# NivekNey/polars-matmul

Hardware: AMD Instinct MI355X
Metric: cosine top-k queries/sec (higher is better)
Workload: dtype f32

## Files before the change

polars-matmul_amd/csrc/pmm_kernels.hip:

```cpp
#include "pmm_device.h"

#include <algorithm>

#include <hip/hip_runtime.h>
#include <math.h>
#include <stdint.h>

#include <type_traits>

namespace pmm {

hipError_t launch_norms_f32(const float *a, int64_t rows, int64_t d, int64_t ld, int squared,
                            float *out, float *inv, hipStream_t s) {
  if (rows <= 0) return hipSuccess;
  const int64_t threads = rows * 8;
  const unsigned grid = (unsigned)((threads + 255) / 256);
  norms_kernel<float><<<grid, 256, 0, s>>>(a, rows, d, ld, squared, out, inv);
  return hipGetLastError();
}
hipError_t launch_norms_pair_f32(const float *q, int64_t m, int64_t ldq, float *qout, const float *c,
                                 int64_t n, int64_t ldc, float *cout, float *cinv, int64_t d, int squared,
                                 hipStream_t s, void *zero, size_t zero_bytes) {
  const unsigned gq = (unsigned)((m * 8 + 255) / 256), gc = (unsigned)((n * 8 + 255) / 256);
  if (zero_bytes % 16 != 0 || ((uintptr_t)zero & 15)) return hipErrorInvalidValue;
// ... 1701 lines not shown
      z1_bytes % 16)
    return hipErrorInvalidValue;
  PrologueArgs a{};
  a.q = q;
  a.ldq = ldq;
  a.m = m;
  a.c = c;
  a.ldc = ldc;
  a.n = n;
  a.d = d;
  a.dp = dp;
  a.ns = ns;
  a.k = k;
  a.squared = metric == kMetricEuclidean;
  a.qn = qn;
  a.cn = cn;
  a.cinv = cn + n;
  a.gthr = gthr;
  a.z0 = (uint4 *)z0;
  a.z1 = (uint4 *)z1;
  a.z0n = (int64_t)(z0_bytes / 16);
  a.z1n = (int64_t)(z1_bytes / 16);
#ifdef PMM_LAB
  a.ablate = getenv("PMM_PROLOGUE_ABLATE") ? atoi(getenv("PMM_PROLOGUE_ABLATE")) : 0;
#endif
  const char *le = getenv("PMM_SEED_LDS");
  a.lds_seed = (ns <= 256 && dp <= seedk::kLdsMaxDp && le && atoi(le) == 1) ? 1 : 0;
  const bool xf = metric != kMetricDot;
  const char *me = getenv("PMM_SEED_MFMA");
  const bool mfma_ok = ns == seedm::NSM && dp <= seedm::kMaxDp && !a.lds_seed && n >= seedm::NSM;
  a.mfma_seed = (mfma_ok && (me ? atoi(me) != 0 : PMM_SEED_MFMA_DEFAULT != 0)) ? 1 : 0;
  if (a.mfma_seed) {
    a.sblocks = (unsigned)((m + seedm::RM - 1) / seedm::RM);
    constexpr int T = seedm::NT;
    a.qblocks = xf ? (unsigned)((m * 8 + T - 1) / T) : 0u;
    a.cblocks = (xf && corpus_norms) ? (unsigned)((n * 8 + T - 1) / T) : 0u;
    a.zblocks = (unsigned)std::max<int64_t>(1, std::min<int64_t>((a.z0n + a.z1n + T - 1) / T, 16));
    const unsigned grid = a.sblocks + a.qblocks + a.cblocks + a.zblocks;
    if (metric == kMetricCosine) return launch_prologue_mfma_t<kMetricCosine>(a, grid, s);
    if (metric == kMetricDot) return launch_prologue_mfma_t<kMetricDot>(a, grid, s);
    return launch_prologue_mfma_t<kMetricEuclidean>(a, grid, s);
  }
  a.sblocks = (unsigned)((m + seedk::RQ - 1) / seedk::RQ);
  unsigned grid;
  if (a.lds_seed) {
    a.qblocks = 0u;
    grid = std::max<unsigned>(a.sblocks, (xf && corpus_norms) ? (unsigned)((n + 63) / 64) : 1u);
    a.cper = (n + grid - 1) / grid;
    a.cblocks = (xf && corpus_norms) ? 1u : 0u;
    a.zblocks = 0u;
  } else {
    a.qblocks = xf ? (unsigned)((m * 8 + 255) / 256) : 0u;
    a.cblocks = (xf && corpus_norms) ? (unsigned)((n * 8 + 255) / 256) : 0u;
    a.zblocks = (unsigned)std::max<int64_t>(1, std::min<int64_t>((a.z0n + a.z1n + 255) / 256, 64));
    grid = a.sblocks + a.qblocks + a.cblocks + a.zblocks;
  }
  if (metric == kMetricCosine) return launch_prologue_t<kMetricCosine>(a, grid, s);
  if (metric == kMetricDot) return launch_prologue_t<kMetricDot>(a, grid, s);
  return launch_prologue_t<kMetricEuclidean>(a, grid, s);
}

constexpr int kMergeRankMaxRows = 16384;
hipError_t launch_merge(const MergeArgs &a0, int loader, hipStream_t s) {
  if (a0.M <= 0) return hipSuccess;
  MergeArgs a = a0;
  static const int rank_env = getenv("PMM_MERGE_RANK") ? atoi(getenv("PMM_MERGE_RANK")) : -1;
  a.no_rank = rank_env == 0 || (rank_env < 0 && a.M > kMergeRankMaxRows);
  a.flags = getenv("PMM_MERGE_FLAGS") ? atoi(getenv("PMM_MERGE_FLAGS"))
                                     : (kMergeReverse | kMergePipelined | kMergeSplitRow);
  const bool sorted = loader == 1 && a.sorted && a.S <= 64 && a.k_out <= 256 && a.P <= 512 &&
                      !(getenv("PMM_MERGE_SORTED") && atoi(getenv("PMM_MERGE_SORTED")) == 0);
  static const int kp = getenv("PMM_KWAY_P") ? atoi(getenv("PMM_KWAY_P")) : 24;
  if (sorted && a.S >= 5 && a.S <= 8 && a.k_out <= 8 * (kp == 32 ? 32 : 24) &&
      !(getenv("PMM_MERGE_KWAY") && atoi(getenv("PMM_MERGE_KWAY")) == 0) &&
      (size_t)MPN(a.P) * 8 <= (size_t)64 * (kp == 32 ? 32 : 24) * 8) {
    static const int wpb = getenv("PMM_KWAY_WPB") ? atoi(getenv("PMM_KWAY_WPB")) : 4;
    const int rows_per_block = 8 * wpb;
    const unsigned grid = (unsigned)((a.M + rows_per_block - 1) / rows_per_block);
    if (kp != 32) {
      if (wpb == 4) (void)hipFuncSetAttribute((const void *)kway_merge_kernel<24>, hipFuncAttributeMaxDynamicSharedMemorySize, 160 * 1024);
      kway_merge_kernel<24><<<grid, 64 * wpb, (size_t)wpb * 64 * 24 * 8, s>>>(a);
    } else {
      if (wpb == 4) (void)hipFuncSetAttribute((const void *)kway_merge_kernel<32>, hipFuncAttributeMaxDynamicSharedMemorySize, 160 * 1024);
      kway_merge_kernel<32><<<grid, 64 * wpb, (size_t)wpb * 64 * 32 * 8, s>>>(a);
    }
    return hipGetLastError();
  }
  if (!(a.S >= 8 && a.k_out <= 64 && a.P <= 512 && !a.no_rank && a.ablate == 0) || sorted) a.flags &= ~kMergeSplitRow;
  const bool split = (a.flags & kMergeSplitRow) != 0;
  int wpb = (int)(65536 / merge_lds_bytes_per_wave(a.P));
  wpb = split ? 4 : (wpb < 1 ? 1 : (wpb > 4 ? 4 : wpb));
  const size_t lds = (size_t)wpb * merge_lds_bytes_per_wave(a.P) + (split ? 16 : 0);
  const unsigned grid = split ? (unsigned)a.M : (unsigned)((a.M + wpb - 1) / wpb);
  if (lds > 65536) {
    static bool attr_set[2] = {false, false};
    if (!attr_set[loader]) {
      const void *fn = loader == 0 ? (const void *)merge_kernel<0, false> : (const void *)merge_kernel<1, false>;
      hipError_t e = hipFuncSetAttribute(fn, hipFuncAttributeMaxDynamicSharedMemorySize, 160 * 1024);
      if (e != hipSuccess) return e;
      attr_set[loader] = true;
    }
  }
  if (sorted) {
    merge_kernel<1, false, true><<<grid, wpb * 64, lds, s>>>(a);
  } else if (split) {
    if (loader == 0) merge_kernel<0, true><<<grid, wpb * 64, lds, s>>>(a);
    else merge_kernel<1, true><<<grid, wpb * 64, lds, s>>>(a);
  } else {
    if (loader == 0) merge_kernel<0, false><<<grid, wpb * 64, lds, s>>>(a);
    else merge_kernel<1, false><<<grid, wpb * 64, lds, s>>>(a);
  }
  return hipGetLastError();
}


template <typename T>
__device__ __forceinline__ u64 score_key(T v, int metric);
template <>
__device__ __forceinline__ u64 score_key<float>(float v, int metric) {
  return (u64)okey32(metric == kMetricEuclidean ? -v : v);
}
template <>
__device__ __forceinline__ u64 score_key<double>(double v, int metric) {
  return okey64(metric == kMetricEuclidean ? -v : v);
}
template <typename T>
__device__ __forceinline__ T key_score(u64 k, int metric);
template <>
__device__ __forceinline__ float key_score<float>(u64 k, int metric) {
  const float v = dekey32((uint32_t)k);
  return metric == kMetricEuclidean ? 0.0f - v : v;
}
template <>
__device__ __forceinline__ double key_score<double>(u64 k, int metric) {
  const double v = dekey64(k);
  return metric == kMetricEuclidean ? 0.0 - v : v;
}

__device__ int ent_compact(Ent *scr, int cnt, int k, int P, Ent *Tv, bool *tfull, int lane) {
  for (int i = cnt + lane; i < P; i += 64) scr[i] = Ent{0ull, 0xFFFFFFFFu, 0u};
  wave_sync();
  wave_sort_desc_ent(scr, P, lane);
  if (cnt >= k) {
    *Tv = scr[k - 1];
    *tfull = true;
    cnt = k;
  }
  wave_sync();
  return cnt;
}

template <typename T>
__global__ __launch_bounds__(256) void rowselect_kernel(RowSelArgs a) {
  extern __shared__ __attribute__((aligned(16))) char smem[];
  const int lane = threadIdx.x & 63, wid = threadIdx.x >> 6;
  const int wpb = blockDim.x >> 6;
  const int row = blockIdx.x * wpb + wid;
  if (row >= a.rows) return;
  Ent *scr = (Ent *)smem + (size_t)wid * a.P;
  const T *src = (const T *)a.scores + (int64_t)row * a.lds;
  Ent Tv{0ull, 0xFFFFFFFFu, 0u};
  bool tfull = false;
  int cnt = 0;
  for (int i0 = 0; i0 < a.N; i0 += 64) {
    const int j = i0 + lane;
    Ent x{0ull, 0xFFFFFFFFu, 0u};
    bool keep = false;
    if (j < a.N) {
      x.key = score_key<T>(src[j], a.metric);
      x.idx = (uint32_t)j;
      keep = !tfull || ent_better(x, Tv);
    }
    const u64 m = __ballot(keep);
    const int pos = cnt + lanes_below(m);
    if (keep) scr[pos] = x;
    cnt += __popcll(m);
    if (cnt > a.P - 64) {
      wave_sync();
      cnt = ent_compact(scr, cnt, a.k, a.P, &Tv, &tfull, lane);
    }
  }
  wave_sync();
  const int P2 = min(a.P, next_pow2_dev(cnt));
  for (int i = cnt + lane; i < P2; i += 64) scr[i] = Ent{0ull, 0xFFFFFFFFu, 0u};
  wave_sync();
  wave_sort_desc_ent(scr, P2, lane);
  T *os = (T *)a.out_score;
  for (int j = lane; j < a.k; j += 64) {
    const Ent x = scr[j];
    a.out_idx[(int64_t)row * a.k + j] = x.idx + a.index_base;
    os[(int64_t)row * a.k + j] = key_score<T>(x.key, a.metric);
  }
}

hipError_t launch_rowselect(const RowSelArgs &a, hipStream_t s) {
  if (a.rows <= 0) return hipSuccess;
  const size_t per_wave = (size_t)a.P * sizeof(Ent);
  int wpb = (int)(65536 / per_wave);
  wpb = wpb < 1 ? 1 : (wpb > 4 ? 4 : wpb);
  const size_t lds = (size_t)wpb * per_wave;
  const unsigned grid = (unsigned)((a.rows + wpb - 1) / wpb);
  if (a.is_f64) rowselect_kernel<double><<<grid, wpb * 64, lds, s>>>(a);
  else rowselect_kernel<float><<<grid, wpb * 64, lds, s>>>(a);
  return hipGetLastError();
}

template <typename T>
__global__ void rowsort_build(const T *__restrict__ scores, int64_t lds, int rows, int N, int P2,
                              int metric, Ent *__restrict__ keys) {
  const int64_t t = (int64_t)blockIdx.x * blockDim.x + threadIdx.x;
  if (t >= (int64_t)rows * P2) return;
  const int r = (int)(t / P2), j = (int)(t % P2);
  Ent e{0ull, 0xFFFFFFFFu, 0u};
  if (j < N) {
    e.key = score_key<T>(scores[(int64_t)r * lds + j], metric);
    e.idx = (uint32_t)j;
  }
  keys[t] = e;
}
__global__ void rowsort_step(Ent *keys, int rows, int P2, int size, int stride) {
  const int64_t t = (int64_t)blockIdx.x * blockDim.x + threadIdx.x;
  const int64_t half = (int64_t)P2 >> 1;
  if (t >= (int64_t)rows * half) return;
  const int r = (int)(t / half), i = (int)(t % half);
  const int x0 = ((i & ~(stride - 1)) << 1) | (i & (stride - 1));
  const int x1 = x0 + stride;
  Ent *base = keys + (int64_t)r * P2;
  const Ent a = base[x0], b = base[x1];
  const bool desc = (x0 & size) == 0;
  if (desc ? ent_better(b, a) : ent_better(a, b)) {
    base[x0] = b;
    base[x1] = a;
  }
}
template <typename T>
__global__ void rowsort_extract(const Ent *__restrict__ keys, int rows, int P2, int k, int metric,
                                uint32_t index_base, uint32_t *__restrict__ out_idx,
                                T *__restrict__ out_score) {
  const int64_t t = (int64_t)blockIdx.x * blockDim.x + threadIdx.x;
  if (t >= (int64_t)rows * k) return;
  const int r = (int)(t / k), j = (int)(t % k);
  const Ent e = keys[(int64_t)r * P2 + j];
  out_idx[t] = e.idx + index_base;
  out_score[t] = key_score<T>(e.key, metric);
}

hipError_t launch_rowsort_global(const void *scores, int64_t lds, int rows, int N, int is_f64,
                                 int metric, void *keys_ws, int P2, int k, uint32_t index_base,
                                 uint32_t *out_idx, void *out_score, hipStream_t s) {
  if (rows <= 0) return hipSuccess;
  Ent *keys = (Ent *)keys_ws;
  const int64_t tot = (int64_t)rows * P2;
  const unsigned gb = (unsigned)((tot + 255) / 256);
  if (is_f64) rowsort_build<double><<<gb, 256, 0, s>>>((const double *)scores, lds, rows, N, P2, metric, keys);
  else rowsort_build<float><<<gb, 256, 0, s>>>((const float *)scores, lds, rows, N, P2, metric, keys);
  const unsigned gs = (unsigned)((tot / 2 + 255) / 256);
  for (int size = 2; size <= P2; size <<= 1)
    for (int stride = size >> 1; stride > 0; stride >>= 1)
      rowsort_step<<<gs, 256, 0, s>>>(keys, rows, P2, size, stride);
  const int64_t tk = (int64_t)rows * k;
  const unsigned ge = (unsigned)((tk + 255) / 256);
  if (is_f64) rowsort_extract<double><<<ge, 256, 0, s>>>(keys, rows, P2, k, metric, index_base, out_idx, (double *)out_score);
  else rowsort_extract<float><<<ge, 256, 0, s>>>(keys, rows, P2, k, metric, index_base, out_idx, (float *)out_score);
  return hipGetLastError();
}

__global__ __launch_bounds__(256) void screen_prep_kernel(const float *__restrict__ rel,
                                                          const unsigned *__restrict__ scal, int m, int dp,
                                                          float *__restrict__ eps, u64 *gthr, int seeded) {
  const int row = (int)(blockIdx.x * blockDim.x + threadIdx.x);
  if (row >= m) return;
  const float e = screen_eps(rel[row], __uint_as_float(scal[0]), dp);
  eps[row] = e;
  if (seeded) gthr[row] = screen_lower(gthr[row], e);
}
hipError_t launch_screen_prep(const float *rel, const unsigned *scal, int m, int dp, float *eps,
                              unsigned long long *gthr, int seeded, hipStream_t s) {
  if (m <= 0) return hipSuccess;
  screen_prep_kernel<<<(unsigned)((m + 255) / 256), 256, 0, s>>>(rel, scal, m, dp, eps, gthr, seeded);
  return hipGetLastError();
}

constexpr int kRescoreList = 512;

template <typename F>
__device__ __forceinline__ void rescore_each_entry(const ScreenFinishArgs &a, u64 *base, const unsigned *segs,
                                                   int nseg, F &&f) {
  const int tid = threadIdx.x, nt = blockDim.x;
  for (int t = 0; t < nseg; t++) {
    const unsigned e = segs[t];
    const int n = (int)(e & 1023u);
    u64 *seg = base + (int64_t)(e >> 10) * a.capg;
    for (int i0 = tid; i0 < n; i0 += 4 * nt) {
      u64 x[4];
#pragma unroll
      for (int j = 0; j < 4; j++) x[j] = i0 + j * nt < n ? seg[i0 + j * nt] : 0ull;
#pragma unroll
      for (int j = 0; j < 4; j++)
        if (i0 + j * nt < n) f(seg + i0 + j * nt, x[j]);
    }
  }
}

__global__ __launch_bounds__(256, 8) void screen_rescore_kernel(ScreenFinishArgs a) {
  extern __shared__ __attribute__((aligned(16))) char smem[];
  __shared__ __attribute__((aligned(16))) unsigned hist[256];
  __shared__ unsigned list[kRescoreList];
  __shared__ unsigned res[4], ln, emin;
  float *qs = (float *)smem;
  unsigned *segs = (unsigned *)(qs + a.dp);
  const int tid = threadIdx.x, nt = blockDim.x;
  const int row = (int)blockIdx.x;
  const float *qr = a.q + (int64_t)row * a.ldq;
  for (int i = 4 * tid; i < a.dp; i += 4 * nt) *(f32x4 *)(qs + i) = *(const f32x4 *)(qr + i);
  for (int i = tid; i < 256; i += nt) hist[i] = 0u;
  if (tid == 0) emin = ~0u, ln = 0u;
  __syncthreads();
  for (int s = tid; s < a.S; s += nt) {
    const unsigned n = min(a.cnt[(int64_t)row * a.S + s], (unsigned)a.capg);
    if (n) segs[atomicAdd(&ln, 1u)] = ((unsigned)s << 10) | n;
  }
  __syncthreads();
  const int nseg = (int)ln;
  const float qv = a.qn[row];
  const float eps = a.eps[row];
  const u64 T = screen_lower(a.gthr[row], eps);
  const u64 T1 = T ? T : 1ull;
  u64 *base = a.cand + (int64_t)row * a.S * a.capg;

  auto live = [&](u64 x) __attribute__((always_inline)) -> bool {
    return x >= T1 && ~(uint32_t)x < (uint32_t)a.N;
  };
  u64 P = 0ull;
  unsigned n_r = 0u, need = (unsigned)a.k;
  for (int shift = 56; shift >= 0; shift -= 8) {
    rescore_each_entry(a, base, segs, nseg, [&](u64 *, u64 x) __attribute__((always_inline)) {
      if (live(x) && (shift == 56 || ((x ^ P) >> (shift + 8)) == 0ull))
        atomicAdd(&hist[(unsigned)(x >> shift) & 255u], 1u);
    });
    __syncthreads();
    if (tid < 64) {
      const uint4 h = ((const uint4 *)hist)[tid];
      ((uint4 *)hist)[tid] = make_uint4(0u, 0u, 0u, 0u);
      const unsigned own = h.x + h.y + h.z + h.w;
      unsigned suf = own;
#pragma unroll
      for (int o = 1; o < 64; o <<= 1) {
        const unsigned t = __shfl_down(suf, o);
        if (tid + o < 64) suf += t;
      }
      if (tid == 0) {
        res[0] = res[1] = res[2] = 0u;
        if (shift == 56) res[3] = suf;
      }
      unsigned above = suf - own;
      if (above < need && suf >= need) {
        unsigned b = 3u, in_bin = h.w;
        if (above + in_bin < need) above += in_bin, in_bin = h.z, b = 2u;
        if (above + in_bin < need) above += in_bin, in_bin = h.y, b = 1u;
        if (above + in_bin < need) above += in_bin, in_bin = h.x, b = 0u;
        res[0] = 4u * (unsigned)tid + b;
        res[1] = need - above;
        res[2] = in_bin;
      }
    }
    __syncthreads();
    P |= (u64)res[0] << shift;
    need = res[1];
    if (shift == 56) n_r = res[3];
    if (res[2] == need) break;
  }
  const int max_rounds = (int)(((int64_t)a.S * a.capg + kRescoreList - 1) / kRescoreList) + 1;
  unsigned done = 0u;
  for (int ph = n_r > (unsigned)a.k ? 1 : 2; ph <= 2; ph++) {
    const bool last = ph == 2;
    u64 thr = P;
    if (last) {
      __syncthreads();
      const u64 E = screen_lower((u64)emin << 32, eps);
      thr = E > T1 ? E : T1;
    }
    for (int r = 0; r < max_rounds; r++) {
      __syncthreads();
      if (tid == 0) ln = 0u;
      __syncthreads();
      rescore_each_entry(a, base, segs, nseg, [&](u64 *p, u64 x) __attribute__((always_inline)) {
        if (x == 0ull) return;
        const uint32_t lw = (uint32_t)x;
        if (!(lw & 0x80000000u)) return;
        if (x < thr || !live(x)) {
          if (last) *p = 0ull;
          return;
        }
        const unsigned pos = atomicAdd(&ln, 1u);
        if (pos < (unsigned)kRescoreList) list[pos] = (unsigned)(p - base);
      });
      __syncthreads();
      const unsigned n = ln;
      const bool more = n > (unsigned)kRescoreList;
      const int cnt = more ? kRescoreList : (int)n;
      for (int t = tid; t < cnt; t += nt) {
        u64 *p = base + list[t];
        const uint32_t col = ~(uint32_t)*p;
        const float *cr = a.c + (int64_t)col * a.ldc;
        float acc = 0.0f;
        for (int k0 = 0; k0 < a.dp; k0 += 32) {
          f32x4 v[8];
#pragma unroll
          for (int j = 0; j < 8; j++) v[j] = *(const f32x4 *)(cr + k0 + 4 * j);
#pragma unroll
          for (int j = 0; j < 8; j++) {
            const f32x4 q4 = *(const f32x4 *)(qs + k0 + 4 * j);
            acc = fmaf(q4[0], v[j][0], acc);
            acc = fmaf(q4[1], v[j][1], acc);
            acc = fmaf(q4[2], v[j][2], acc);
            acc = fmaf(q4[3], v[j][3], acc);
          }
        }
        const uint32_t key = okey32(exact_score<kMetricCosine>(acc, qv, a.cn[col]));
        if (!last) atomicMin(&emin, key);
        *p = ((u64)key << 32) | (u64)col;
        done++;
      }
      if (!more) break;
    }
  }
  __syncthreads();
  rescore_each_entry(a, base, segs, nseg, [&](u64 *p, u64 x) __attribute__((always_inline)) {
    if (x != 0ull && !((uint32_t)x & 0x80000000u)) *p = (x & 0xFFFFFFFF00000000ull) | (u64)(~(uint32_t)x);
  });
  if (a.stat) {
    __syncthreads();
    if (tid == 0) ln = 0u;
    __syncthreads();
    atomicAdd(&ln, done);
    __syncthreads();
    if (tid == 0) {
      atomicAdd(a.stat, ln);
      atomicMax(a.stat + 1, ln);
      atomicAdd(a.stat + 2, n_r);
    }
  }
}
hipError_t launch_screen_rescore(const ScreenFinishArgs &a, hipStream_t s) {
  if (a.M <= 0) return hipSuccess;
  if (a.dp % 32 != 0 || a.dp > 4096 || a.ldq % 4 != 0 || a.ldc % 4 != 0 || a.ldq < a.dp || a.ldc < a.dp ||
      (((uintptr_t)a.q | (uintptr_t)a.c) & 15) || a.k < 1 || a.k > kRescoreList || a.capg > 1023 ||
      ((int64_t)a.dp + a.S) * 4 > 64 * 1024)
    return hipErrorInvalidValue;
  int nt = 64;
  if (const char *e = getenv("PMM_RESCORE_BLOCK")) {
    const int v = atoi(e);
    if (v == 64 || v == 128 || v == 256) nt = v;
  }
  screen_rescore_kernel<<<(unsigned)a.M, nt, ((size_t)a.dp + a.S) * 4, s>>>(a);
  return hipGetLastError();
}

__device__ __forceinline__ bool is_pos_zero(float v) { return __float_as_uint(v) == 0u; }
__device__ __forceinline__ bool is_pos_zero(double v) { return __double_as_longlong(v) == 0ll; }
__device__ __forceinline__ float fma_chain_step(float a, float b, float c) { return fmaf(a, b, c); }
__device__ __forceinline__ double fma_chain_step(double a, double b, double c) { return __fma_rn(a, b, c); }
__device__ __forceinline__ float cosine_of(float dot, float qv, float cv) {
  return exact_score<kMetricCosine>(dot, qv, cv);
}
__device__ __forceinline__ double cosine_of(double dot, double qv, double cv) {
  return exact_score_f64<kMetricCosine>(dot, qv, cv);
}
template <typename T>
__global__ __launch_bounds__(256) void zero_sign_kernel(const T *__restrict__ q, int64_t ldq,
                                                        const T *__restrict__ c, int64_t ldc,
                                                        const T *__restrict__ qn, const T *__restrict__ cn,
                                                        int m, int64_t n, int d, int k, int metric,
                                                        uint32_t index_base, const uint32_t *__restrict__ out_idx,
                                                        T *__restrict__ out_score) {
  const int64_t t = (int64_t)blockIdx.x * blockDim.x + threadIdx.x;
  if (t >= (int64_t)m * k) return;
  if (!is_pos_zero(out_score[t])) return;
  const uint32_t id = out_idx ? out_idx[t] : (uint32_t)(t % k) + index_base;
  if (id == 0xFFFFFFFFu) return;
  const int64_t col = (int64_t)(uint32_t)(id - index_base);
  if (col >= n) return;
  const int row = (int)(t / k);
  const T *qr = q + (int64_t)row * ldq, *cr = c + col * ldc;
  T acc = (T)0;
  for (int i = 0; i < d; i++) acc = fma_chain_step(qr[i], cr[i], acc);
  const T sc = metric == kMetricDot ? acc : cosine_of(acc, qn[row], cn[col]);
  if (sc == (T)0) out_score[t] = sc;
}
hipError_t launch_zero_sign_f32(const float *q, int64_t ldq, const float *c, int64_t ldc, const float *qn,
                                const float *cn, int m, int64_t n, int d, int k, int metric, uint32_t index_base,
                                const uint32_t *out_idx, float *out_score, hipStream_t s) {
  if (m <= 0 || k <= 0 || metric == kMetricEuclidean) return hipSuccess;
  zero_sign_kernel<float><<<(unsigned)(((int64_t)m * k + 255) / 256), 256, 0, s>>>(
      q, ldq, c, ldc, qn, cn, m, n, d, k, metric, index_base, out_idx, out_score);
  return hipGetLastError();
}
hipError_t launch_zero_sign_f64(const double *q, int64_t ldq, const double *c, int64_t ldc, const double *qn,
                                const double *cn, int m, int64_t n, int d, int k, int metric, uint32_t index_base,
                                const uint32_t *out_idx, double *out_score, hipStream_t s) {
  if (m <= 0 || k <= 0 || metric == kMetricEuclidean) return hipSuccess;
  zero_sign_kernel<double><<<(unsigned)(((int64_t)m * k + 255) / 256), 256, 0, s>>>(
      q, ldq, c, ldc, qn, cn, m, n, d, k, metric, index_base, out_idx, out_score);
  return hipGetLastError();
}

__global__ __launch_bounds__(256) void zero_sign_lists_kernel(const uint32_t *__restrict__ in_idx,
                                                              const float *__restrict__ in_score, int lists,
                                                              int k_in, int64_t row_stride, int64_t list_stride,
                                                              int m, int k, const uint32_t *__restrict__ out_idx,
                                                              float *__restrict__ out_score) {
  const int64_t t = (int64_t)blockIdx.x * blockDim.x + threadIdx.x;
  if (t >= (int64_t)m * k) return;
  if (__float_as_uint(out_score[t]) != 0u) return;
  const uint32_t id = out_idx[t];
  if (id == 0xFFFFFFFFu) return;
  const int64_t row = t / k;
  for (int g = 0; g < lists; g++) {
    const int64_t base = (int64_t)g * list_stride + row * row_stride;
    for (int j = 0; j < k_in; j++) {
      if (in_idx[base + j] != id) continue;
      const float sc = in_score[base + j];
      if (sc == 0.0f) out_score[t] = sc;
      return;
    }
  }
}
hipError_t launch_zero_sign_lists(const uint32_t *in_idx, const float *in_score, int lists, int k_in,
                                  int64_t row_stride, int64_t list_stride, int m, int k, const uint32_t *out_idx,
                                  float *out_score, hipStream_t s) {
  if (m <= 0 || k <= 0 || lists <= 0) return hipSuccess;
  zero_sign_lists_kernel<<<(unsigned)(((int64_t)m * k + 255) / 256), 256, 0, s>>>(
      in_idx, in_score, lists, k_in, row_stride, list_stride, m, k, out_idx, out_score);
  return hipGetLastError();
}

__global__ __launch_bounds__(256) void screen_collect_kernel(const unsigned *__restrict__ ovf,
                                                             const unsigned *__restrict__ bad, int m,
                                                             unsigned *count, int *__restrict__ rows) {
  const int row = (int)(blockIdx.x * blockDim.x + threadIdx.x);
  if (row < m && (ovf[row] | bad[row])) {
    rows[atomicAdd(count, 1u)] = row;
    if (ovf[row]) atomicAdd(count + 1, 1u);
  }
}
hipError_t launch_screen_collect(const unsigned *ovf, const unsigned *bad, int m, unsigned *count, int *rows,
                                 hipStream_t s) {
  if (m <= 0) return hipSuccess;
  screen_collect_kernel<<<(unsigned)((m + 255) / 256), 256, 0, s>>>(ovf, bad, m, count, rows);
  return hipGetLastError();
}

__global__ __launch_bounds__(256) void gather_rows_kernel(const uint4 *__restrict__ src, int64_t ld,
                                                          const int *__restrict__ rows, int r, int units,
                                                          uint4 *__restrict__ dst) {
  const int64_t t = (int64_t)blockIdx.x * blockDim.x + threadIdx.x;
  if (t >= (int64_t)r * units) return;
  const int i = (int)(t / units), c = (int)(t - (int64_t)i * units);
  dst[t] = src[(int64_t)rows[i] * ld + c];
}
hipError_t launch_gather_rows(const void *src, int64_t ld_units, const int *rows, int r, int units, void *dst,
                              hipStream_t s) {
  if (r <= 0 || units <= 0) return hipSuccess;
  gather_rows_kernel<<<(unsigned)(((int64_t)r * units + 255) / 256), 256, 0, s>>>((const uint4 *)src, ld_units, rows,
                                                                                  r, units, (uint4 *)dst);
  return hipGetLastError();
}
__global__ __launch_bounds__(256) void scatter_lists_kernel(const uint32_t *__restrict__ oi,
                                                            const float *__restrict__ os,
                                                            const int *__restrict__ rows, int r, int k,
                                                            uint32_t *__restrict__ out_idx,
                                                            float *__restrict__ out_score) {
  const int64_t t = (int64_t)blockIdx.x * blockDim.x + threadIdx.x;
  if (t >= (int64_t)r * k) return;
  const int i = (int)(t / k), j = (int)(t - (int64_t)i * k);
  out_idx[(int64_t)rows[i] * k + j] = oi[t];
  out_score[(int64_t)rows[i] * k + j] = os[t];
}
hipError_t launch_scatter_lists(const uint32_t *oi, const float *os, const int *rows, int r, int k,
                                uint32_t *out_idx, float *out_score, hipStream_t s) {
  if (r <= 0) return hipSuccess;
  scatter_lists_kernel<<<(unsigned)(((int64_t)r * k + 255) / 256), 256, 0, s>>>(oi, os, rows, r, k, out_idx,
                                                                               out_score);
  return hipGetLastError();
}

}
```

Before: 610,300.

## Add register-resident single-wave rescore fast path for single-segment rows

Adds a fast path in the screen rescore kernel for rows whose candidates sit in one segment of at most 512 entries. When the block is a single 64-thread wave, those candidates are held in registers. Filtering and selection use wave ballots and a wave k-th selection in place of the repeated shared-memory radix-histogram passes and atomics. Dot-product scoring is factored into a helper, and launch bounds drop from 8 to 6 blocks per CU to give the register array room, at some cost to occupancy. The path can be disabled with an environment variable.

```diff
diff --git a/polars-matmul_amd/csrc/pmm_kernels.hip b/polars-matmul_amd/csrc/pmm_kernels.hip
--- a/polars-matmul_amd/csrc/pmm_kernels.hip
+++ b/polars-matmul_amd/csrc/pmm_kernels.hip
@@ -2027,7 +2027,78 @@
   }
 }
 
-__global__ __launch_bounds__(256, 8) void screen_rescore_kernel(ScreenFinishArgs a) {
+__device__ __forceinline__ uint32_t rescore_key(const ScreenFinishArgs &a, const float *qs, float qv, uint32_t col) {
+  const float *cr = a.c + (int64_t)col * a.ldc;
+  float acc = 0.0f;
+  for (int k0 = 0; k0 < a.dp; k0 += 32) {
+    f32x4 v[8];
+#pragma unroll
+    for (int j = 0; j < 8; j++) v[j] = *(const f32x4 *)(cr + k0 + 4 * j);
+#pragma unroll
+    for (int j = 0; j < 8; j++) {
+      const f32x4 q4 = *(const f32x4 *)(qs + k0 + 4 * j);
+      acc = fmaf(q4[0], v[j][0], acc);
+      acc = fmaf(q4[1], v[j][1], acc);
+      acc = fmaf(q4[2], v[j][2], acc);
+      acc = fmaf(q4[3], v[j][3], acc);
+    }
+  }
+  return okey32(exact_score<kMetricCosine>(acc, qv, a.cn[col]));
+}
+
+__device__ __forceinline__ unsigned rescore_row_regs(const ScreenFinishArgs &a, u64 *seg, u64 (&x)[8], const float *qs,
+                                                     float qv, float eps, u64 T1, unsigned short *lslot,
+                                                     unsigned *lcol, unsigned &n_r) {
+  const int lane = threadIdx.x;
+  int live_n = 0;
+#pragma unroll
+  for (int e = 0; e < 8; e++) {
+    const bool live = x[e] >= T1 && ~(uint32_t)x[e] < (uint32_t)a.N;
+    if (x[e] != 0ull && !live) seg[lane + 64 * e] = 0ull;
+    if (!live) x[e] = 0ull;
+    live_n += __popcll(__ballot(live));
+  }
+  n_r = (unsigned)live_n;
+  uint32_t kmin = ~0u;
+  unsigned done = 0u;
+  auto pass = [&](u64 thr, bool last) __attribute__((always_inline)) {
+    int cnt = 0;
+#pragma unroll
+    for (int e = 0; e < 8; e++) {
+      const bool wait = x[e] != 0ull, keep = wait && x[e] >= thr;
+      const u64 m = __ballot(keep);
+      if (keep) {
+        const int pos = cnt + lanes_below(m);
+        lslot[pos] = (unsigned short)(lane + 64 * e);
+        lcol[pos] = ~(uint32_t)x[e];
+      } else if (wait && last) {
+        seg[lane + 64 * e] = 0ull;
+      }
+      if (keep) x[e] = 0ull;
+      cnt += __popcll(m);
+    }
+    __syncthreads();
+    for (int t = lane; t < cnt; t += 64) {
+      const uint32_t col = lcol[t];
+      const uint32_t key = rescore_key(a, qs, qv, col);
+      seg[lslot[t]] = ((u64)key << 32) | (u64)(~col);
+      if (!last) kmin = key < kmin ? key : kmin;
+      done++;
+    }
+    __syncthreads();
+  };
+  if (live_n > a.k) pass(wave_kth_u64<8>(x, a.k), false);
+#pragma unroll
+  for (int o = 32; o; o >>= 1) {
+    const uint32_t w = (uint32_t)__shfl_xor((int)kmin, o);
+    kmin = w < kmin ? w : kmin;
+  }
+  const u64 E = screen_lower((u64)kmin << 32, eps);
+  pass(E > T1 ? E : T1, true);
+  return done;
+}
+
+__global__ __launch_bounds__(256, 6) void screen_rescore_kernel(ScreenFinishArgs a, int regs) {
   extern __shared__ __attribute__((aligned(16))) char smem[];
   __shared__ __attribute__((aligned(16))) unsigned hist[256];
   __shared__ unsigned list[kRescoreList];
@@ -2037,6 +2108,38 @@
   const int tid = threadIdx.x, nt = blockDim.x;
   const int row = (int)blockIdx.x;
   const float *qr = a.q + (int64_t)row * a.ldq;
+  u64 *base = a.cand + (int64_t)row * a.S * a.capg;
+  if (regs && nt == 64 && a.S <= 64) {
+    const unsigned n = tid < a.S ? min(a.cnt[(int64_t)row * a.S + tid], (unsigned)a.capg) : 0u;
+    const u64 m = __ballot(n != 0u);
+    if (__popcll(m) == 1) {
+      const int sg = __builtin_ctzll(m);
+      const int n1 = (int)wave_uniform_u32((uint32_t)__shfl((int)n, sg));
+      if (n1 <= 512) {
+        u64 *seg = base + (int64_t)sg * a.capg;
+        u64 x[8];
+#pragma unroll
+        for (int e = 0; e < 8; e++) x[e] = tid + 64 * e < n1 ? seg[tid + 64 * e] : 0ull;
+        for (int i = 4 * tid; i < a.dp; i += 4 * 64) *(f32x4 *)(qs + i) = *(const f32x4 *)(qr + i);
+        const float eps = a.eps[row];
+        const u64 T = screen_lower(a.gthr[row], eps);
+        __syncthreads();
+        unsigned n_r;
+        unsigned done = rescore_row_regs(a, seg, x, qs, a.qn[row], eps, T ? T : 1ull, (unsigned short *)hist, list,
+                                         n_r);
+        if (a.stat) {
+#pragma unroll
+          for (int o = 32; o; o >>= 1) done += (unsigned)__shfl_xor((int)done, o);
+          if (tid == 0) {
+            atomicAdd(a.stat, done);
+            atomicMax(a.stat + 1, done);
+            atomicAdd(a.stat + 2, n_r);
+          }
+        }
+        return;
+      }
+    }
+  }
   for (int i = 4 * tid; i < a.dp; i += 4 * nt) *(f32x4 *)(qs + i) = *(const f32x4 *)(qr + i);
   for (int i = tid; i < 256; i += nt) hist[i] = 0u;
   if (tid == 0) emin = ~0u, ln = 0u;
@@ -2051,7 +2154,6 @@
   const float eps = a.eps[row];
   const u64 T = screen_lower(a.gthr[row], eps);
   const u64 T1 = T ? T : 1ull;
-  u64 *base = a.cand + (int64_t)row * a.S * a.capg;
 
   auto live = [&](u64 x) __attribute__((always_inline)) -> bool {
     return x >= T1 && ~(uint32_t)x < (uint32_t)a.N;
@@ -2127,22 +2229,7 @@
       for (int t = tid; t < cnt; t += nt) {
         u64 *p = base + list[t];
         const uint32_t col = ~(uint32_t)*p;
-        const float *cr = a.c + (int64_t)col * a.ldc;
-        float acc = 0.0f;
-        for (int k0 = 0; k0 < a.dp; k0 += 32) {
-          f32x4 v[8];
-#pragma unroll
-          for (int j = 0; j < 8; j++) v[j] = *(const f32x4 *)(cr + k0 + 4 * j);
-#pragma unroll
-          for (int j = 0; j < 8; j++) {
-            const f32x4 q4 = *(const f32x4 *)(qs + k0 + 4 * j);
-            acc = fmaf(q4[0], v[j][0], acc);
-            acc = fmaf(q4[1], v[j][1], acc);
-            acc = fmaf(q4[2], v[j][2], acc);
-            acc = fmaf(q4[3], v[j][3], acc);
-          }
-        }
-        const uint32_t key = okey32(exact_score<kMetricCosine>(acc, qv, a.cn[col]));
+        const uint32_t key = rescore_key(a, qs, qv, col);
         if (!last) atomicMin(&emin, key);
         *p = ((u64)key << 32) | (u64)col;
         done++;
@@ -2178,7 +2265,9 @@
     const int v = atoi(e);
     if (v == 64 || v == 128 || v == 256) nt = v;
   }
-  screen_rescore_kernel<<<(unsigned)a.M, nt, ((size_t)a.dp + a.S) * 4, s>>>(a);
+  const char *rp = getenv("PMM_RESCORE_PATH");
+  const int regs = !(rp && atoi(rp) == 0);
+  screen_rescore_kernel<<<(unsigned)a.M, nt, ((size_t)a.dp + a.S) * 4, s>>>(a, regs);
   return hipGetLastError();
 }
 
```

Result: no change. 614,600 (median of 6 runs) (+0.7%).
